# projecthorus/radiosonde_auto_rx

Hardware: AMD Instinct MI355X
Metric: IQ Msamples/s (RS41 --IQ --lpIQ demod + framesync + ECC), concurrent real-time 2.4 Msps channels = value/2.4 (higher is better)
Workload: dtype f32; 1 GPU; RS41 2.4 Msps cs16 IQ, rs41mod --ecc2 --IQ fq --lpIQ (BASELINE configs[1]) x 512 channels per GPU (per-GPU share of configs[4]), 1 s of signal per channel per step, input resident in HBM; channels_per_gpu=512, frames_decoded=507392, frames_ecc_ok=457842, frames_ecc_failed=49550, frames_repaired=200182, symbols_repaired=1815512

## Files before the change

include/sonde_hip.h:

```cpp
#ifndef SONDE_HIP_H
#define SONDE_HIP_H

#include <stdint.h>
#include <stddef.h>

#ifdef __cplusplus
extern "C" {
#endif

#define SONDE_ABI_VERSION 3

#define SONDE_E_ARG      (-1)
#define SONDE_E_NOGPU    (-2)
#define SONDE_E_NOMEM    (-3)
#define SONDE_E_RANGE    (-4)
#define SONDE_E_OVERFLOW (-5)

#define SONDE_RS41  41
#define SONDE_FRONTEND 0
#define SONDE_DFM09  9
#define SONDE_M10    10
#define SONDE_M20    20

#define SONDE_RD94RD41 94
// ... 109 lines not shown
int64_t sonde_engine_samples_to_dc_boundary(const sonde_engine_t *e);
int  sonde_engine_sync(sonde_engine_t *e);

typedef struct {
    uint32_t channel_id;
    uint8_t  type;
    uint8_t  inverted;
    uint16_t reserved;
    float    score;
    float    freq_offset_hz;
    uint64_t sample_pos;
    uint32_t frames;
    uint32_t frames_clean;
} sonde_summary_t;
int  sonde_engine_set_summary(sonde_engine_t *e, void *d_summary, uint32_t channel_base);
int  sonde_engine_set_summary_snapshots(sonde_engine_t *e, void *d_snap);

int  sonde_engine_fetch_frames(sonde_engine_t *e, sonde_frame_t *out, int32_t max);
int  sonde_engine_overflowed(sonde_engine_t *e);
long long sonde_engine_host_ecc_frames(sonde_engine_t *e);
int  sonde_engine_set_device_ecc(sonde_engine_t *e, int32_t on);
int  sonde_engine_set_search_rounds(sonde_engine_t *e, int32_t on);
int  sonde_engine_count_windows(sonde_engine_t *e, int32_t on, int64_t *out);
int  sonde_engine_read_sync_state(sonde_engine_t *e, uint32_t *out, int32_t max_channels);
int  sonde_engine_fetch_frames_lagged(sonde_engine_t *e, sonde_frame_t *out, int32_t max, int32_t lag);

typedef struct {
    int32_t  channel;
    int32_t  nbits;
    uint32_t mv_pos;
    float    mv;
} sonde_hit_t;
int  sonde_engine_fetch_hits(sonde_engine_t *e, sonde_hit_t *out, int32_t max, int32_t finish);
int  sonde_engine_set_sync(sonde_engine_t *e, int32_t hdmax, int32_t bitofs);
int  sonde_engine_fetch_soft1(sonde_engine_t *e, float *soft, int32_t max_frames);
int  sonde_engine_set_threshold(sonde_engine_t *e, float thres);

int  sonde_engine_fetch_dfm(sonde_engine_t *e, sonde_dfm_frame_t *out, int32_t max, int32_t finish);
int  sonde_engine_fetch_dfm_lagged(sonde_engine_t *e, sonde_dfm_frame_t *out, int32_t max, int32_t lag);
typedef struct {
    int32_t  channel;
    int32_t  nbits;
    int32_t  len;
    int32_t  cs_ok;
    uint32_t cs_calc;
    uint32_t mv_pos;
// ... 73 lines not shown
```

radiosonde_auto_rx_amd/csrc/sonde_dev.h:

```cpp
#ifndef SONDE_DEV_H
#define SONDE_DEV_H
#include <hip/hip_runtime.h>
#include <stdint.h>
#include "../../include/sonde_hip.h"

struct MixDecArgs {
    const int16_t *iq;
    long long ch_stride;
    int n_ch, nblocks;
    int D, Q;
    int G;
    int wgs_per_ch;
    float wtab[64 * 8];
    const double *chan_f0;
    int lut_len;
    uint32_t lut_phase;
    const float2 *dc_avg;
    long long *dc_sums;
    const float2 *ptail_in;
    float2 *ptail_out;
    float2 *y;
    int ring_len;
    uint32_t m0;
    const float *wtab_g;
// ... 157 lines not shown
int  sonde_launch_framesync_multi(const SyncArgs *a, int n_groups, hipStream_t s);
int  sonde_launch_mix_decimate(const MixDecArgs *a, hipStream_t s);
void sonde_launch_dc_update(int n_ch, long long *sums, float2 *avg, float maxcnt, hipStream_t s);
void sonde_launch_dc_update_keep(int n_ch, long long *sums, float2 *avg, float2 *avg_prev, float maxcnt, hipStream_t s);
void sonde_launch_publish_u32(const unsigned *src, unsigned *dst_mapped, hipStream_t s);
void sonde_launch_dc_update_pcs(int n_ch, long long *sums, float2 *avg, float2 *avg_prev, uint32_t *cnt, uint32_t *max, uint32_t lim, int32_t *since,
                                uint32_t n_samples, int nblocks, hipStream_t s);
void sonde_launch_md_etable(const double *chan_f0, const float *wtab, int D, int Q, int P, int n_ch, float2 *etab, hipStream_t s);
void sonde_launch_if_chain(const IfArgs *a, hipStream_t s);
void sonde_launch_mix_f32(const MixF32Args *a, hipStream_t s);
void sonde_launch_dc_segments_f32(const float2 *x, long long ch_stride, int n_ch, int n_samples, unsigned dc_cnt0, unsigned dc_max,
                                  double *seg_sums, double *dc_sums, float2 *dc_avg, float2 *dc_seg, int dc_seg_n, hipStream_t s);
void sonde_launch_decimate_f32(const DecF32Args *a, hipStream_t s);
void sonde_launch_dc_update_f64(int n_ch, double *sums, float2 *avg, float maxcnt, hipStream_t s);
void sonde_launch_afc_rotate(const AfcRotArgs *a, hipStream_t s, int n_max);
void sonde_launch_fill_u32(uint32_t *p, uint32_t v, int n, hipStream_t s);
void sonde_launch_audio_chain(const AudioChainArgs *a, hipStream_t s);
void sonde_launch_u8_to_s16(const uint8_t *in, long long in_stride, int16_t *out, long long out_stride, int n_ch, int n_bytes, hipStream_t s);
void sonde_launch_header_corr(const CorrArgs *a, hipStream_t s);
void sonde_launch_sync_plan(const WinPlanArgs *a, hipStream_t s);
void sonde_launch_sync_window_fft(const WinFftArgs *a, hipStream_t s);
void sonde_launch_framesync(const SyncArgs *a, hipStream_t s);
void sonde_launch_search_sync(const SearchSyncArgs *a, hipStream_t s);
}
#endif
```

radiosonde_auto_rx_amd/csrc/sonde_engine.cpp:

```cpp
#include "../../include/sonde_hip.h"
#include "sonde_dev.h"
#include "sonde_host.h"
#include "sonde_scan_dev.h"
#include <algorithm>
#include <cmath>
#include <cstdio>
#include <cstring>
#include <map>
#include <string>
#include <vector>

using namespace sonde;

#define HIPCHK(x) do { hipError_t e_ = (x); if (e_ != hipSuccess) { fprintf(stderr, "libsonde_hip: %s failed: %s\n", #x, hipGetErrorString(e_)); return SONDE_E_NOGPU; } } while (0)

struct KernelStat { double ms = 0; int64_t n = 0; };
struct PendingEvt { hipEvent_t a, b; const char *name; };

struct sonde_engine {
    sonde_cfg_t cfg{};
    sonde_info_t info{};
    hipStream_t stream = nullptr;
    hipStream_t stream_b = nullptr;
    unsigned long long *d_wfprof = nullptr;
// ... 761 lines not shown
            hipMemcpyAsync(e->d_summary_snap + (size_t)(e->call & 1) * C, e->d_summary, (size_t)C * sizeof(sonde_summary_t), hipMemcpyDeviceToDevice, e->stream_b);
            hipEventRecord(e->ev_b[slot], e->stream_b);
            e->snap_calls = e->call + 1;
        }
        e->call += 1;
    } else {
        if (e->stream_b != e->stream) hipEventRecord(e->ev_a[slot], e->stream);
        rc = tail_enqueue(e, n_samples, m_first, e->stream, e->ev_a[slot]);
    }
    return rc;
}

}

static IfArgs fill_if(sonde_engine *e, int n_if, uint32_t m_first) {
    IfArgs b{};
    const bool fe = e->cfg.sonde_type == SONDE_FRONTEND;
    b.y = e->d_y; b.tap_ifiq = (e->cfg.keep_soft || fe) ? e->d_ifiq : nullptr; b.fm = e->d_fm; b.bufs = e->d_bufs; b.n_ch = e->cfg.n_channels; b.ring_len = e->ring_len;
    b.n = n_if; b.m0 = m_first;
    b.lpiq_on = !e->w_iq.empty(); b.lpiq_taps = (int)e->w_iq.size(); b.lpfm_on = !e->w_fm.empty(); b.lpfm_taps = (int)e->w_fm.size();
    b.tone_on = (e->cfg.input != SONDE_IN_IFIQ0); b.nwin = (int)e->sps;
    b.fm_on = (e->cfg.keep_soft || fe || !e->w_fm.empty() || !b.tone_on) ? 1 : 0;
    b.w_iq = e->d_wiq; b.w_fm = e->d_wfm; b.rho = e->rho; b.sps = e->sps; b.epoch = e->d_epoch;
    return b;
}
static int tail_enqueue(sonde_engine *e, int32_t n_samples, uint32_t m_first, hipStream_t fs, hipEvent_t front_done) {
    const int D = e->info.decM, C = e->cfg.n_channels;
    const int n_if = n_samples / D;
    const bool fe = e->cfg.sonde_type == SONDE_FRONTEND;
    IfArgs b = fill_if(e, n_if, m_first);
    const int slot = (int)(e->call & 3);
    if (e->stream_b != fs) hipStreamWaitEvent(e->stream_b, front_done, 0);
    CorrArgs c{};
    c.bufs = e->d_bufs; c.corr = e->d_corr; c.match = e->d_match; c.n_ch = C; c.ring_len = e->ring_len; c.n = n_if; c.L = e->info.L; c.m0 = m_first;
    c.state = e->d_state; c.delay = e->info.delay; c.frame_samples = e->frame_samples;
    c.ntypes = e->corr_types; c.isps = e->corr_isps; c.nsym = e->hdrlen / e->symhd; c.shapes = e->d_shapes; c.sym_type = e->d_symtype; c.sym_sign = e->d_symsign;
    if (e->cfg.opt_dc && e->cfg.input != SONDE_IN_AUDIO) {
        hipStream_t sb = e->stream_b;
        sonde_launch_fill_u32(e->d_start, m_first, C, sb);
        b.y = e->d_yrot; b.tap_ifiq = e->d_ifiq; b.afc = e->d_afc; b.start = e->d_start; b.fmraw = e->d_fmraw; b.w_iq0 = e->d_wiq0; b.fm_on = 1;
        c.start = e->d_start;
        AfcRotArgs r{}; r.y = e->d_y; r.yrot = e->d_yrot; r.afc = e->d_afc; r.start = e->d_start; r.n_ch = C; r.ring_len = e->ring_len;
        r.sr = e->info.if_sr; r.m_end = e->m_out;
        for (int it = 0; it < n_if / std::max(1, e->info.K - 4) + 4; it++) {
            hipMemsetAsync(e->d_pending, 0, sizeof(unsigned), sb);
            sonde_launch_afc_rotate(&r, sb, n_if);
            prof_begin(e, "if_chain", sb); sonde_launch_if_chain(&b, sb); prof_end(e, sb);
            prof_begin(e, "header_corr", sb); sonde_launch_header_corr(&c, sb); prof_end(e, sb);
            if (e->opt_iq >= 2) { CorrArgs c2 = c; c2.bufs = e->d_fm; c2.corr = e->d_corr2; sonde_launch_header_corr(&c2, sb); }
            launch_framesync(e, 0);
            hipMemcpyAsync(e->h_pending, e->d_pending, sizeof(unsigned), hipMemcpyDeviceToHost, sb);
            HIPCHK(hipStreamSynchronize(sb));
            if (*e->h_pending == 0) break;
        }
        if (e->stream_b != fs) hipEventRecord(e->ev_if[slot], e->stream_b);
    } else {
        if (e->cfg.input != SONDE_IN_AUDIO) { prof_begin(e, "if_chain", e->stream_b); sonde_launch_if_chain(&b, e->stream_b); prof_end(e, e->stream_b); }
        if (e->stream_b != fs) hipEventRecord(e->ev_if[slot], e->stream_b);
        if (!fe && e->d_win && !e->search_rounds) {
            launch_search_sync(e);
        } else if (!fe && e->d_win) {
            const int rounds = sync_rounds_of(e, n_if);
            for (int round = 0; round < rounds; round++) {
// ... 217 lines not shown
    if (!e) return SONDE_E_ARG;
    long long n = e->host_ecc_frames;
    for (sonde_engine *g : e->groups) n += g->host_ecc_frames;
    return n;
}
int sonde_engine_set_search_rounds(sonde_engine_t *e, int32_t on) {
    if (!e) return SONDE_E_ARG;
    for (sonde_engine *g : e->groups) { const int rc = sonde_engine_set_search_rounds(g, on); if (rc) return rc; }
    e->search_rounds = on != 0;
    return 0;
}
int sonde_engine_count_windows(sonde_engine_t *e, int32_t on, int64_t *out) {
    if (!e || !e->groups.empty()) return SONDE_E_ARG;
    if (on && !e->d_wcount && e->d_win && dalloc(&e->d_wcount, 1)) return SONDE_E_NOMEM;
    if (hipStreamSynchronize(e->stream_b) != hipSuccess) return SONDE_E_NOGPU;
    e->count_windows = on != 0;
    if (out) {
        unsigned long long n = 0;
        if (e->d_wcount && hipMemcpy(&n, e->d_wcount, sizeof n, hipMemcpyDeviceToHost) != hipSuccess) return SONDE_E_NOGPU;
        out[0] = e->wcount_rounds[0]; out[1] = e->wcount_rounds[1]; out[2] = (int64_t)n;
    }
    return 0;
}
int sonde_engine_read_sync_state(sonde_engine_t *e, uint32_t *out, int32_t max_channels) {
    if (!e || !out || !e->groups.empty() || !e->d_state) return SONDE_E_ARG;
    const int n = std::min<int>(max_channels, e->cfg.n_channels);
    if (n <= 0) return 0;
    if (hipStreamSynchronize(e->stream_b) != hipSuccess) return SONDE_E_NOGPU;
    if (hipMemcpy(out, e->d_state, (size_t)n * sizeof(SyncState), hipMemcpyDeviceToHost) != hipSuccess) return SONDE_E_NOGPU;
    return n;
}
int sonde_engine_set_device_ecc(sonde_engine_t *e, int32_t on) {
    if (!e) return SONDE_E_ARG;
    for (sonde_engine *g : e->groups) { const int rc = sonde_engine_set_device_ecc(g, on); if (rc) return rc; }
    if ((on != 0) == e->dev_ecc) return 0;
    if (e->d_blk_done) {
        if (hipStreamSynchronize(e->stream_b) != hipSuccess) return SONDE_E_NOGPU;
        unsigned count = 0;
        if (hipMemcpy(&count, e->d_fcount, sizeof count, hipMemcpyDeviceToHost) != hipSuccess) return SONDE_E_NOGPU;
        if (count != e->read_idx) return SONDE_E_ARG;
        const unsigned dn[2] = { count, 0u };
        if (on && hipMemcpy(e->d_blk_done, dn, sizeof dn, hipMemcpyHostToDevice) != hipSuccess) return SONDE_E_NOGPU;
    }
    e->dev_ecc = on != 0;
    return 0;
}
// ... 478 lines not shown
```

radiosonde_auto_rx_amd/csrc/sonde_kernels.hip:

```cpp
#include <hip/hip_runtime.h>
#include <stdint.h>
#include "sonde_dev.h"
#include "md_fast_gen.h"
#include "sonde_rs_dev.h"
#include <cstdlib>

typedef short  short2v __attribute__((ext_vector_type(2)));

#define WAVE 64

#define MD_ROWS   64
#define MD_NVMAX  16

struct __attribute__((packed, aligned(4))) u32x4_u { uint32_t x, y, z, w; };

typedef float float2v __attribute__((ext_vector_type(2)));

__device__ __forceinline__ float2v cmul_pk(float2v u, float2v cs) {
    float2v t, z;
    asm("s_nop 0\n\tv_pk_mul_f32 %0, %1, %2 op_sel:[1,1] op_sel_hi:[1,0] neg_lo:[0,1]" : "=&v"(t) : "v"(u), "v"(cs));
    asm("v_pk_fma_f32 %0, %1, %2, %3 op_sel_hi:[0,1,1]" : "=&v"(z) : "v"(u), "v"(cs), "v"(t));
    return z;
}

template <int Q_T, bool WRAP, bool PH64>
__device__ __forceinline__ void md_step(const uint32_t raw, const int r, const float *w, const float2v navg, const float2v msk,
                                        const double f0, double &ndrun, const uint32_t rown, const uint32_t towrap, const uint32_t L,
                                        float2v (&acc)[Q_T], float2v &dcs) {
// ... 1031 lines not shown
        yr[m & mask] = r;
    }
}

__global__ void k_fill_u32(uint32_t *p, uint32_t v, int n) {
    const int i = blockIdx.x * blockDim.x + threadIdx.x;
    if (i < n) p[i] = v;
}

#ifndef IF_TILE
#define IF_TILE 960
#endif
#ifndef IF_THREADS
#define IF_THREADS 256
#endif
#ifndef IF_NB
#define IF_NB 4
#endif
#define IF_RUN 4
#ifndef IF_LD
#define IF_LD 5
#endif

__device__ __forceinline__ void if_chain_body(const IfArgs &a, const int ch, const int bx) {
    extern __shared__ __attribute__((aligned(16))) float smem[];
    const uint32_t t0 = a.m0 + (uint32_t)bx * IF_TILE;
    const int nout = min(IF_TILE, (int)(a.m0 + (uint32_t)a.n - t0));
    if (nout <= 0) return;
    const bool afc = a.afc != nullptr;
    const uint32_t start = afc ? a.start[ch] : t0;
    if (afc && (int32_t)(t0 + (uint32_t)nout - start) <= 0) return;
    const uint32_t mask = (uint32_t)a.ring_len - 1;
    const int T1 = a.lpiq_on ? a.lpiq_taps : 1;
    const int T2 = a.lpfm_on ? a.lpfm_taps : 1;
    const int nwin = a.nwin;
    const int64_t ep = a.epoch ? (int64_t)a.epoch[ch] : 0;
    const int hz = (T2 - 1) + max(1, nwin - 1);
    const int nz = hz + nout;
    const int ny = nz + (T1 - 1);
    const int nyp = (ny + 2 * IF_NB + 1) & ~1;
    float2 *sy = reinterpret_cast<float2 *>(smem);
    const int nzs = a.fm_on ? nz + (nz & 1) : 0;
    float2 *sz = sy + nyp;
    float4 *sx4 = reinterpret_cast<float4 *>(sz + nzs);
    float  *sf = reinterpret_cast<float *>(sx4 + (a.tone_on ? nz : 0));
    const int nsf = a.fm_on ? T2 - 1 + nout : 0;
    float  *wf = sf + nsf;
    float  *wq = sf + ((nsf + T2 + 3) & ~3);

    const float2 *yr = a.y + (size_t)ch * a.ring_len;
    for (int kb = threadIdx.x; kb < nyp; kb += IF_LD * IF_THREADS) {
        float2 v[IF_LD];
#pragma unroll
        for (int u = 0; u < IF_LD; u++) {
            const int k = kb + u * IF_THREADS;
            const int64_t m = (int64_t)t0 - hz - (T1 - 1) + k;
            v[u] = (m >= 0 && k < ny) ? yr[(uint32_t)m & mask] : make_float2(0.f, 0.f);
        }
#pragma unroll
        for (int u = 0; u < IF_LD; u++) { const int k = kb + u * IF_THREADS; if (k < nyp) sy[k] = v[u]; }
    }
    const int acq = __builtin_amdgcn_readfirstlane((afc && !a.afc[ch].locked) ? 1 : 0);
    const float *w_iq = acq ? a.w_iq0 : a.w_iq;
    for (int k = threadIdx.x; k < T2; k += IF_THREADS) wf[k] = a.lpfm_on ? a.w_fm[k] : 1.0f;
    for (int k = threadIdx.x; k < T1; k += IF_THREADS) wq[k] = a.lpiq_on ? w_iq[k] : 1.0f;
    typedef const float __attribute__((address_space(4))) *cfptr;
    const cfptr wtaps = (cfptr)(uintptr_t)w_iq;
    __syncthreads();

    typedef float v2f __attribute__((ext_vector_type(2)));
    for (int k0 = IF_NB * threadIdx.x; k0 < nz; k0 += IF_NB * IF_THREADS) {
        v2f acc[IF_NB];
#pragma unroll
        for (int j = 0; j < IF_NB; j++) acc[j] = v2f{0.f, 0.f};
        v2f win[IF_NB + 2];
#pragma unroll
        for (int j = 0; j < IF_NB; j += 2) {
            const float4 v0 = *reinterpret_cast<const float4 *>(sy + k0 + j);
            win[j] = v2f{v0.x, v0.y}; win[j + 1] = v2f{v0.z, v0.w};
        }
        int t = 0;
#ifdef IF_EXP_NOFIR
        t = T1 & ~3;
#endif
        for (; t + 3 < T1; t += 4) {
            const float4 n0 = *reinterpret_cast<const float4 *>(sy + k0 + t + IF_NB), n1 = *reinterpret_cast<const float4 *>(sy + k0 + t + IF_NB + 2);
            const float4 w4 = make_float4(wtaps[t], wtaps[t + 1], wtaps[t + 2], wtaps[t + 3]);
            win[IF_NB] = v2f{n0.x, n0.y}; win[IF_NB + 1] = v2f{n0.z, n0.w};
#pragma unroll
            for (int j = 0; j < IF_NB; j++) {
                acc[j] = __builtin_elementwise_fma(win[j], v2f{w4.x, w4.x}, acc[j]);
                acc[j] = __builtin_elementwise_fma(win[j + 1], v2f{w4.y, w4.y}, acc[j]);
            }
// ... 29 lines not shown
#pragma unroll
            for (int j = 0; j < IF_NB; j++) acc[j] = __builtin_elementwise_fma(win[j], v2f{w0, w0}, acc[j]);
        }
#pragma unroll
        for (int j = 0; j < IF_NB; j++) {
            const int k = k0 + j;
            if (k >= nz) break;
            float re = acc[j].x, im = acc[j].y;
            const int64_t m = (int64_t)t0 - hz + k;
            if (m < 0) { re = 0.f; im = 0.f; }
            else if (afc && (int32_t)((uint32_t)m - start) < 0) {
                const float2 zo = a.tap_ifiq[(size_t)ch * a.ring_len + ((uint32_t)m & mask)];
                re = zo.x; im = zo.y;
            }
            if (a.fm_on) sz[k] = make_float2(re, im);
            if (a.tone_on) {
#ifdef IF_EXP_NOTONE
                const float sn = 0.f, cs = 1.f;
#else
                const float fr = (float)__builtin_amdgcn_fract((double)(m - ep) * a.rho);
                const float sn = __builtin_amdgcn_sinf(fr), cs = __builtin_amdgcn_cosf(fr);
#endif
                const float rc = re * cs, ic = im * cs;
                sx4[k] = make_float4(__builtin_fmaf(-sn, im, rc), __builtin_fmaf(sn, re, ic), __builtin_fmaf(sn, im, rc), __builtin_fmaf(-sn, re, ic));
            }
            if (a.tap_ifiq && m >= (int64_t)t0 && (int32_t)((uint32_t)m - start) >= 0)
                a.tap_ifiq[(size_t)ch * a.ring_len + ((uint32_t)m & mask)] = make_float2(re, im);
        }
    }
    __syncthreads();

    if (a.fm_on)
    for (int k = threadIdx.x; k < T2 - 1 + nout; k += IF_THREADS) {
        const int zi = k + (hz - (T2 - 1));
        const float2 z1 = sz[zi], z0 = sz[zi - 1];
        const float wr = z1.x * z0.x + z1.y * z0.y, wi = z1.y * z0.x - z1.x * z0.y;
#ifdef IF_EXP_NOATAN
        float v = wi + wr;
#else
        float v = 0.8f * atan2f(wi, wr) * 0.31830988618379067f;
#endif
        if (afc) {
            const int64_t m = (int64_t)t0 - (T2 - 1) + k;
            float *fr = a.fmraw + (size_t)ch * a.ring_len;
            if (m >= 0 && (int32_t)((uint32_t)m - start) < 0) v = fr[(uint32_t)m & mask];
            else if (m >= (int64_t)t0) fr[(uint32_t)m & mask] = v;
        }
        sf[k] = v;
    }
    __syncthreads();

    float *bufs = a.bufs + (size_t)ch * a.ring_len;
    float *fmb = a.fm + (size_t)ch * a.ring_len;
    const float inv_sps = 1.0f / a.sps;
    for (int k0 = IF_RUN * threadIdx.x; k0 < nout; k0 += IF_RUN * IF_THREADS) {
        float4 f = make_float4(0.f, 0.f, 0.f, 0.f);
        float so[IF_RUN], sfm[IF_RUN];
        const bool vec = !afc && k0 + IF_RUN <= nout && ((t0 + (uint32_t)k0) & (IF_RUN - 1)) == 0;
#pragma unroll
        for (int r = 0; r < IF_RUN; r++) {
            const int k = k0 + r;
            so[r] = 0.f; sfm[r] = 0.f;
            if (k >= nout) break;
            const uint32_t m = t0 + (uint32_t)k;
            if (a.tone_on) {
#ifdef IF_EXP_NOWIN
                if (1) { f = sx4[hz + k]; } else
#endif
                if (r == 0) {
                    for (int j = nwin - 1; j >= 0; j--) { const float4 x = sx4[hz + k - j]; f.x += x.x; f.y += x.y; f.z += x.z; f.w += x.w; }
                } else {
                    const float4 xn = sx4[hz + k], xo = sx4[hz + k - nwin];
                    f.x += xn.x - xo.x; f.y += xn.y - xo.y; f.z += xn.z - xo.z; f.w += xn.w - xo.w;
                }
            }
            if (afc && (int32_t)(m - start) < 0) continue;
            float s_fm = 0.f;
            if (a.fm_on) {
                s_fm = sf[T2 - 1 + k];
                if (a.lpfm_on) {
                    float acc = 0.f;
                    for (int t = 0; t < T2; t++) acc = fmaf(sf[k + t], wf[t], acc);
                    s_fm = acc;
                }
                if (!vec) fmb[m & mask] = s_fm;
            }
            float s = s_fm;
            if (a.tone_on) s = (__builtin_amdgcn_sqrtf(f.z * f.z + f.w * f.w) - __builtin_amdgcn_sqrtf(f.x * f.x + f.y * f.y)) * inv_sps;
            if (!vec) bufs[m & mask] = s;
            so[r] = s; sfm[r] = s_fm;
        }
        if (vec) {
            const uint32_t mi = (t0 + (uint32_t)k0) & mask;
            static_assert(IF_RUN == 4, "the vector store below writes four outputs");
            *reinterpret_cast<float4 *>(bufs + mi) = make_float4(so[0], so[1], so[2], so[3]);
            if (a.fm_on) *reinterpret_cast<float4 *>(fmb + mi) = make_float4(sfm[0], sfm[1], sfm[2], sfm[3]);
        }
    }
}

__global__ __launch_bounds__(IF_THREADS)
void k_if_chain(const IfArgs a) { if_chain_body(a, blockIdx.y, blockIdx.x); }
template <class A> struct MultiArgs { A g[SONDE_MAX_GROUPS]; int row0[SONDE_MAX_GROUPS + 1]; int n_groups; };
template <class A> __device__ __forceinline__ int multi_group(const MultiArgs<A> &m, const int row) {
    int g = 0;
    while (g + 1 < m.n_groups && row >= m.row0[g + 1]) g++;
    return __builtin_amdgcn_readfirstlane(g);
}
__global__ __launch_bounds__(IF_THREADS)
void k_if_chain_multi(const MultiArgs<IfArgs> m) {
    const int g = multi_group(m, (int)blockIdx.y);
    if_chain_body(m.g[g], (int)blockIdx.y - m.row0[g], blockIdx.x);
}

__device__ __forceinline__ uint32_t sync_first_pos(const SyncState &st, uint32_t frame_samples, int delay) {
    uint32_t first;
    if (st.mode == 1) first = st.mv_pos + 1 + frame_samples;
    else first = st.s_in - st.k;
    return first - (uint32_t)(delay + 16);
}
__device__ __forceinline__ bool corr_tile_unused(const CorrArgs &a, int ch, uint32_t tile_start, uint32_t tile_end) {
    if (a.start && (int32_t)(tile_end - a.start[ch]) <= 0) return true;
    if (!a.state) return false;
    const SyncState st = a.state[ch];
    if (st.mode != 0 && st.mode != 1) return true;
    const uint32_t first = sync_first_pos(st, a.frame_samples, a.delay);
    if (a.limit && (int32_t)(tile_start - (first + a.limit)) >= 0) return true;
    return (int32_t)(tile_end - first) <= 0;
}

#define HC_TILE 1024
#define HC_THREADS 256
// ... 83 lines not shown
    float *corr = a.corr + (size_t)ch * a.ring_len;
#if HCF_TILE / HCF_THREADS >= 2
    for (int o2 = threadIdx.x * 2; o2 < HCF_TILE; o2 += 2 * HCF_THREADS) {
        float c0 = 0.f, c1 = 0.f;
        for (int k = 0; k < nsym; k++) {
            const int ty = a.sym_type[k];
            const float sg = a.sym_sign[k];
            const float2 u = *reinterpret_cast<const float2 *>(sF + ty * nf + sps * k + o2);
            c0 = fmaf(sg, u.x, c0); c1 = fmaf(sg, u.y, c1);
        }
        if (o2 < nout) corr[(p0 + (uint32_t)o2) & mask] = c0;
        if (o2 + 1 < nout) corr[(p0 + (uint32_t)(o2 + 1)) & mask] = c1;
    }
#else
    {
        const int o = threadIdx.x;
        float c0 = 0.f;
        for (int k = 0; k < nsym; k++) c0 = fmaf(a.sym_sign[k], sF[a.sym_type[k] * nf + sps * k + o], c0);
        if (o < nout) corr[(p0 + (uint32_t)o) & mask] = c0;
    }
#endif
}

__device__ __forceinline__ float wave_sum(float v) {
    for (int off = 32; off > 0; off >>= 1) v += __shfl_xor(v, off);
    return v;
}

__device__ __forceinline__ void bit_window(int pos, int half, int symlen, float sps,
                                           uint32_t &q0, uint32_t &q1, double &mid) {
    double bg = (pos == 0) ? 0.0 : (double)((float)(pos * symlen) * sps);
    double prev;
    if (half == 0) {
        if (pos == 0) prev = 0.0;
        else {
            prev = (pos == 1) ? 0.0 : (double)((float)((pos - 1) * symlen) * sps);
            prev += (double)sps;
            if (symlen == 2) prev += (double)sps;
        }
    } else {
        bg += (double)sps;
        prev = bg;
    }
    q0 = (uint32_t)ceil(prev);
    mid = bg + (double)(sps - 1.0f) / 2.0;
    q1 = (uint32_t)ceil(bg + (double)sps);
// ... 90 lines not shown
    __syncthreads();
    float c = corr[mpos & mask];
    if (DC) c -= off;
    mv = c / sqrtf(e);
    return bidx;
}

struct NoWinEval {
    static constexpr bool fused = false;
    __device__ int operator()(int, uint32_t, float &, uint32_t &) const { return -4; }
};
template <bool DC, int NT = FS_THREADS, class Eval = NoWinEval>
__device__ __forceinline__ void framesync_body(const SyncArgs &a, const int ch, const Eval &eval = Eval{}) {
    __shared__ uint8_t s_frame[520];
    __shared__ uint8_t s_exp[512];
    __shared__ uint8_t s_log[256];
    __shared__ float s_rf[(NT / WAVE)];
    __shared__ int s_ri[(NT / WAVE)];
    __shared__ int s_cnt[2];
    __shared__ unsigned s_slot;
    __shared__ uint8_t s_syn[(NT / WAVE)][48];
    __shared__ uint8_t s_S[48];
    __shared__ double s_rd[(NT / WAVE)];
    const int tid = threadIdx.x, lane = tid & 63, wave = tid >> 6;
    if (ch >= a.n_ch) return;
    const uint32_t mask = (uint32_t)a.ring_len - 1;
    const float *bufs = a.bufs + (size_t)ch * a.ring_len;
    const float *corr = a.corr + (size_t)ch * a.ring_len;
    SyncState st = a.state[ch];
    const uint32_t ep = a.epoch ? a.epoch[ch] : 0u;
    uint32_t avail = a.avail;
    AfcState af{};
    if (DC) af = a.afc[ch];
    bool afc_event = false;
    const int K = a.K, L = a.L;

#define FS_MARK(k) do { if (a.prof && ch == 0 && tid == 0) { const unsigned long long t_ = __builtin_readcyclecounter(); a.prof[k] += t_ - t_prev; t_prev = t_; } } while (0)
    unsigned long long t_prev = a.prof ? __builtin_readcyclecounter() : 0ull;
    for (int i = tid; i < 512; i += NT) s_exp[i] = a.gf_exp[i];
    for (int i = tid; i < 256; i += NT) s_log[i] = a.gf_log[i];
    __syncthreads();
    FS_MARK(0);
    const bool horizon_on = a.corr_limit != 0 && (st.mode == 0 || st.mode == 1);
    const uint32_t horizon = horizon_on ? sync_first_pos(st, a.frame_samples, a.delay) + a.corr_limit : 0u;

    for (int guard = 0; guard < (1 << 20); guard++) {
        if (st.mode == 2) break;
        if (st.mode == 0) {
            const uint32_t need = (uint32_t)(K - 4) - st.k;
            const uint32_t s_in_w = st.s_in + need;
            if ((int32_t)(avail - s_in_w) < 0) { st.k += avail - st.s_in; st.s_in = avail; break; }
            if (horizon_on && (int32_t)(s_in_w - 1 - (uint32_t)a.delay - horizon) >= 0) break;
            const uint32_t pos = s_in_w - 1 - (uint32_t)a.delay;
            const WinItem *wi = nullptr;
            if (!DC && !Eval::fused && a.win && pos >= (uint32_t)L) {
                for (int w = 0; w < a.win_W; w++) { const WinItem *c = a.win + (size_t)ch * a.win_W + w; if (c->state == 2 && c->pos == pos) { wi = c; break; } }
                if (!wi) break;
            }
            st.s_in = s_in_w; st.k = 0; st.mv = 0.f;
            if (pos - ep < (uint32_t)L) continue;
            float mv; uint32_t mpos;
            if (wi) { if (wi->rc < 0) { if (wi->rc == -5) st.mv_pos = wi->mpos; continue; } mv = wi->mv; mpos = wi->mpos; }
            else if (Eval::fused && pos >= (uint32_t)L) {
                const int rc = eval(ch, pos, mv, mpos);
                if (rc < 0) { if (rc == -5) st.mv_pos = mpos; continue; }
            } else {
                const int rc = fs_window<DC, NT>(bufs, corr, mask, pos, K, L, a.N, a.match_sum, tid, lane, wave, s_rf, s_ri, mv, mpos);
                if (rc == -5) { st.mv_pos = mpos; if (DC) af.dc = 0.0; }
                if (rc < 0) continue;
            }
// ... 263 lines not shown
#define WF_THREADS 512
#endif
#define FFT_THREADS WF_THREADS
#include "sonde_fft_dev.h"
#ifndef WF_MB
#define WF_MB 4
#endif
#ifndef WF_LU
#define WF_LU 1
#endif
#ifndef WF_LB
#define WF_LB 4
#endif
#define WF_MARK(k) do { if (a.prof && blockIdx.x == 0 && tid == 0) { const unsigned long long t_ = __builtin_readcyclecounter(); a.prof[k] += t_ - t_prev; t_prev = t_; } } while (0)
struct WinItemIo {
    static constexpr int copy = 0;
    WinItem *it;
    __device__ bool planned() const { return it->state == 1; }
    __device__ uint32_t pos() const { return it->pos; }
    __device__ void put(int rc, float mv, uint32_t mpos) const { it->rc = rc; it->mv = mv; it->mpos = mpos; __threadfence(); it->state = 2; }
};
template <class Io>
__device__ __forceinline__ void sync_eval_window(const WinFftArgs &a, const int ch, const Io &io, float2 *x, float2 *tws, float *s_rf, int *s_ri) {
    const int tid = threadIdx.x, lane = tid & 63, wave = tid >> 6;
    if (!io.planned()) return;
    unsigned long long t_prev = a.prof ? __builtin_readcyclecounter() : 0ull;
    const int K = a.K, L = a.L, N = SC_N, wl = K + L;
    const uint32_t pos = io.pos(), mask = (uint32_t)a.ring_len - 1;
    const float *bufs = a.bufs + (size_t)ch * a.ring_len;
    const int64_t start = (int64_t)pos - (wl - 1);
    {
        constexpr int NL = SC_N / WF_THREADS;
#pragma unroll 1
        for (int h = 0; h < NL; h += WF_LB) {
            float v[WF_LB];
#pragma unroll
            for (int u = 0; u < WF_LB; u++) {
                const int i = tid + (h + u) * WF_THREADS;
                const int64_t p = start + i;
                v[u] = (i < wl && p >= 0) ? bufs[(uint32_t)p & mask] : 0.f;
            }
#pragma unroll
            for (int u = 0; u < WF_LB; u++) x[XI(brev13(tid + (h + u) * WF_THREADS))] = make_float2(v[u], 0.f);
        }
    }
    __syncthreads();
    WF_MARK(0);
    dft_ref<Io::copy>(x, tws, a.tws, tid);
    WF_MARK(1);
    {
        const float2 *FmR = a.Fm + N;
#pragma unroll 1
        for (int h = 0; h < N / WF_THREADS; h += WF_MB) {
            float2 fi[WF_MB], fr[WF_MB];
#pragma unroll
            for (int u = 0; u < WF_MB; u++) {
                const int i = tid + (h + u) * WF_THREADS;
                const bool on = brev13(i) >= i;
                fi[u] = on ? a.Fm[i] : make_float2(0.f, 0.f);
                fr[u] = on ? FmR[i] : make_float2(0.f, 0.f);
            }
#pragma unroll
            for (int u = 0; u < WF_MB; u++) {
                const int i = tid + (h + u) * WF_THREADS, r = brev13(i);
                if (r < i) continue;
                const float2 zi = cmul(x[XI(i)], fi[u]), zr = cmul(x[XI(r)], fr[u]);
                x[XI(r)] = make_float2(zi.x, -zi.y);
                x[XI(i)] = make_float2(zr.x, -zr.y);
            }
        }
    }
    __syncthreads();
    WF_MARK(2);
    dft_ref_head<Io::copy>(x, tws, a.tws, tid);
    float best = 0.f, bestc = 0.f; int bidx = -1;
#pragma unroll WF_LU
    for (int u = 0; u < SC_N / 2 / WF_THREADS; u++) {
        const int g = tid + u * WF_THREADS;
        const float2 w = a.tws[((1 << 12) - 1) + g];
        const float2 p = x[XI(g)], r = cmul(x[XI(g + (1 << 12))], w);
        const float c0 = p.x + r.x, c1 = p.x - r.x;
        const int i0 = g, i1 = g + (1 << 12);
        if (i0 >= L - 1 && i0 < wl) { const float c2 = c0 * c0; if (c2 > best || (c2 == best && bidx >= 0 && i0 < bidx)) { best = c2; bidx = i0; bestc = c0; } }
        if (i1 >= L - 1 && i1 < wl) { const float c2 = c1 * c1; if (c2 > best || (c2 == best && bidx >= 0 && i1 < bidx)) { best = c2; bidx = i1; bestc = c1; } }
    }
    WF_MARK(3);
    {
        float rb = best; int ri = bidx;
        for (int off = 32; off > 0; off >>= 1) {
            const float ob = __shfl_xor(rb, off); const int oi = __shfl_xor(ri, off);
            if (ob > rb || (ob == rb && oi >= 0 && (ri < 0 || oi < ri))) { rb = ob; ri = oi; }
        }
        if (lane == 0) { s_rf[wave] = rb; s_ri[wave] = ri; }
    }
    __syncthreads();
    int mp = -1;
// ... 215 lines not shown
extern "C" void sonde_launch_decimate_f32(const DecF32Args *a, hipStream_t s) {
    if (a->nblocks <= 0) return;
    int jper = DF32_J;
    auto lds_of = [&](int j) { return (size_t)(a->D * (j - 1) + a->T) * sizeof(float2) + (size_t)a->T * sizeof(float); };
    while (jper > 8 && lds_of(jper) > 64 * 1024) jper >>= 1;
    if (lds_of(jper) > 64 * 1024) { hipLaunchKernelGGL(k_decimate_f32_global, dim3((a->nblocks + 255) / 256, a->n_ch), dim3(256), 0, s, *a); return; }
    hipLaunchKernelGGL(k_decimate_f32, dim3((a->nblocks + jper - 1) / jper, a->n_ch), dim3(DF32_J), lds_of(jper), s, *a, jper);
}
extern "C" void sonde_launch_dc_update_f64(int n_ch, double *sums, float2 *avg, float maxcnt, hipStream_t s) {
    hipLaunchKernelGGL(k_dc_update_f64, dim3((n_ch + 255) / 256), dim3(256), 0, s, n_ch, sums, avg, maxcnt);
}
extern "C" void sonde_launch_afc_rotate(const AfcRotArgs *a, hipStream_t s, int n_max) {
    int gx = (n_max + 255) / 256; if (gx > 256) gx = 256; if (gx < 1) gx = 1;
    hipLaunchKernelGGL(k_afc_rotate, dim3(gx, a->n_ch), dim3(256), 0, s, *a);
}
extern "C" void sonde_launch_fill_u32(uint32_t *p, uint32_t v, int n, hipStream_t s) {
    hipLaunchKernelGGL(k_fill_u32, dim3((n + 255) / 256), dim3(256), 0, s, p, v, n);
}
extern "C" void sonde_launch_audio_chain(const AudioChainArgs *a, hipStream_t s) {
    int gx = (a->n + 255) / 256; if (gx > 256) gx = 256; if (gx < 1) gx = 1;
    hipLaunchKernelGGL(k_audio_chain, dim3(gx, a->n_ch), dim3(256), 0, s, *a);
}
extern "C" void sonde_launch_if_chain(const IfArgs *a, hipStream_t s) {
    const int T1 = a->lpiq_on ? a->lpiq_taps : 1, T2 = a->lpfm_on ? a->lpfm_taps : 1;
    const int hz = (T2 - 1) + (a->nwin - 1 > 1 ? a->nwin - 1 : 1);
    const int nz = hz + IF_TILE, ny = nz + T1 - 1;
    const size_t lds = (size_t)((ny + 2 * IF_NB + 1) & ~1) * 8 + (size_t)(a->fm_on ? nz + 1 : 0) * 8 + (size_t)(a->tone_on ? nz : 0) * 16 + (size_t)(a->fm_on ? T2 - 1 + IF_TILE : 0) * 4 + (size_t)(T1 + T2) * 4 + 32;
    hipLaunchKernelGGL(k_if_chain, dim3((a->n + IF_TILE - 1) / IF_TILE, a->n_ch), dim3(IF_THREADS), lds, s, *a);
}
template <class A> static MultiArgs<A> multi_pack(const A *a, const int *rows, int n_groups) {
    MultiArgs<A> m{};
    m.n_groups = n_groups; m.row0[0] = 0;
    for (int g = 0; g < n_groups; g++) { m.g[g] = a[g]; m.row0[g + 1] = m.row0[g] + rows[g]; }
    return m;
}
static_assert(sizeof(MultiArgs<IfArgs>) <= 4096, "MultiArgs<IfArgs> exceeds the kernel argument segment");
static_assert(sizeof(MultiArgs<WinPlanArgs>) <= 4096, "MultiArgs<WinPlanArgs> exceeds the kernel argument segment");
static_assert(sizeof(MultiArgs<WinFftArgs>) <= 4096, "MultiArgs<WinFftArgs> exceeds the kernel argument segment");
static_assert(sizeof(MultiArgs<SyncArgs>) <= 4096, "MultiArgs<SyncArgs> exceeds the kernel argument segment");
extern "C" int sonde_launch_if_chain_multi(const IfArgs *a, int n_groups, hipStream_t s) {
    if (n_groups < 1 || n_groups > SONDE_MAX_GROUPS) return -1;
    size_t lds = 0; int rows[SONDE_MAX_GROUPS], n = a[0].n;
    for (int g = 0; g < n_groups; g++) {
        const int T1 = a[g].lpiq_on ? a[g].lpiq_taps : 1, T2 = a[g].lpfm_on ? a[g].lpfm_taps : 1;
        const int hz = (T2 - 1) + (a[g].nwin - 1 > 1 ? a[g].nwin - 1 : 1);
        const int nz = hz + IF_TILE, ny = nz + T1 - 1;
        const size_t l = (size_t)((ny + 2 * IF_NB + 1) & ~1) * 8 + (size_t)(a[g].fm_on ? nz + 1 : 0) * 8 + (size_t)(a[g].tone_on ? nz : 0) * 16 + (size_t)(a[g].fm_on ? T2 - 1 + IF_TILE : 0) * 4 + (size_t)(T1 + T2) * 4 + 32;
        if (l > lds) lds = l;
        rows[g] = a[g].n_ch;
        if (a[g].n != n) return -1;
    }
    const MultiArgs<IfArgs> m = multi_pack(a, rows, n_groups);
    hipLaunchKernelGGL(k_if_chain_multi, dim3((n + IF_TILE - 1) / IF_TILE, m.row0[n_groups]), dim3(IF_THREADS), lds, s, m);
    return 0;
}
extern "C" int sonde_launch_sync_plan_multi(const WinPlanArgs *a, int n_groups, hipStream_t s) {
    if (n_groups < 1 || n_groups > SONDE_MAX_GROUPS) return -1;
    int rows[SONDE_MAX_GROUPS];
    for (int g = 0; g < n_groups; g++) rows[g] = a[g].n_ch;
    const MultiArgs<WinPlanArgs> m = multi_pack(a, rows, n_groups);
    hipLaunchKernelGGL(k_sync_plan_multi, dim3((m.row0[n_groups] + 255) / 256), dim3(256), 0, s, m);
    return 0;
}
extern "C" int sonde_launch_sync_window_fft_multi(const WinFftArgs *a, int n_groups, hipStream_t s) {
    if (n_groups < 1 || n_groups > SONDE_MAX_GROUPS) return -1;
    long long tot = 0; int rows[SONDE_MAX_GROUPS];
    for (int g = 0; g < n_groups; g++) tot += (long long)a[g].W * a[g].n_ch;
    const long long cap = tot > 512 ? 512 : tot;
    for (int g = 0; g < n_groups; g++) { const long long w = (long long)a[g].W * a[g].n_ch; rows[g] = (int)((w * cap + tot - 1) / tot); if (rows[g] < 1) rows[g] = 1; }
    const MultiArgs<WinFftArgs> m = multi_pack(a, rows, n_groups);
// ... 78 lines not shown
    if (tid == 0) { ecc[f] = r; codes[2 * f] = L.res[0]; codes[2 * f + 1] = L.res[1]; }
}
extern "C" void sonde_launch_rs41_ecc_batch(uint8_t *frames, const int32_t *flen, int n, int level, int32_t *ecc, int32_t *codes, uint8_t *synd,
                                            const uint8_t *gf_exp, const uint8_t *gf_log, hipStream_t s) {
    hipLaunchKernelGGL(k_rs41_ecc_batch, dim3(n), dim3(RSK_THREADS), 0, s, frames, flen, level, ecc, codes, synd, gf_exp, gf_log, (const unsigned *)nullptr);
}
extern "C" void sonde_launch_rs41_ecc_batch_n(uint8_t *frames, const int32_t *flen, const unsigned *count, int cap, int level, int32_t *ecc, int32_t *codes, uint8_t *synd,
                                              const uint8_t *gf_exp, const uint8_t *gf_log, hipStream_t s) {
    hipLaunchKernelGGL(k_rs41_ecc_batch, dim3(cap), dim3(RSK_THREADS), 0, s, frames, flen, level, ecc, codes, synd, gf_exp, gf_log, count);
}

extern "C" int sonde_launch_framesync_multi(const SyncArgs *a, int n_groups, hipStream_t s) {
    if (n_groups < 1 || n_groups > SONDE_MAX_GROUPS) return -1;
    int rows[SONDE_MAX_GROUPS];
    for (int g = 0; g < n_groups; g++) { rows[g] = a[g].n_ch; if (a[g].opt_dc) return -1; }
    const MultiArgs<SyncArgs> m = multi_pack(a, rows, n_groups);
    hipLaunchKernelGGL(k_framesync_multi, dim3(m.row0[n_groups]), dim3(1024), 0, s, m);
    return 0;
}
extern "C" void sonde_launch_framesync(const SyncArgs *a, hipStream_t s) {
    if (a->opt_dc) hipLaunchKernelGGL(k_framesync<true>, dim3(a->n_ch), dim3(FS_THREADS), 0, s, *a);
    else hipLaunchKernelGGL(k_framesync<false>, dim3(a->n_ch), dim3(FS_THREADS), 0, s, *a);
}
extern "C" void sonde_launch_search_sync(const SearchSyncArgs *a, hipStream_t s) {
    const size_t lds = (size_t)(SC_XN + SC_TW_LDS + 1) * sizeof(float2);
    hipLaunchKernelGGL(k_search_sync, dim3(a->sync.n_ch), dim3(WF_THREADS), lds, s, *a);
}
```

radiosonde_auto_rx_amd/engine.py:

```python
from __future__ import annotations

import ctypes as C
import os
import subprocess

import numpy as np

_HERE = os.path.dirname(os.path.abspath(__file__))
LIB_PATH = os.environ.get("SONDE_HIP_LIB", os.path.join(_HERE, "libsonde_hip.so"))

SONDE_RS41 = 41
SONDE_DFM09 = 9
SONDE_M10 = 10
SONDE_RD94RD41 = 94
SONDE_M20 = 20
LP_IQ, LP_FM = 1, 2
TAP_DECIM, TAP_IFIQ, TAP_FM, TAP_BUFS, TAP_CORR = range(5)
ABI_VERSION = 3


class SondeCfg(C.Structure):
    _fields_ = [(n, C.c_int32) for n in ("abi_version", "device", "n_channels", "sample_rate", "bits", "sonde_type",
                                         "opt_lp", "opt_dc", "opt_min", "lpiq_bw", "ecc_level")] + \
               [("thres", C.c_float), ("max_chunk", C.c_int32), ("max_frames", C.c_int32), ("keep_soft", C.c_int32),
# ... 199 lines not shown
    def set_summary(self, device_ptr: int, channel_base: int = 0):
        _chk(lib().sonde_engine_set_summary(self._h, C.c_void_p(device_ptr), channel_base))

    def set_summary_snapshots(self, device_ptr: int) -> int:
        return _chk(lib().sonde_engine_set_summary_snapshots(self._h, C.c_void_p(device_ptr)))

    def overflowed(self) -> bool:
        return bool(_chk(lib().sonde_engine_overflowed(self._h)))

    def host_ecc_frames(self) -> int:
        return int(lib().sonde_engine_host_ecc_frames(self._h))

    def set_device_ecc(self, on: bool):
        _chk(lib().sonde_engine_set_device_ecc(self._h, 1 if on else 0))

    def set_search_rounds(self, on: bool):
        _chk(lib().sonde_engine_set_search_rounds(self._h, 1 if on else 0))

    def count_windows(self, on: bool = True):
        out = np.zeros(3, dtype=np.int64)
        _chk(lib().sonde_engine_count_windows(self._h, 1 if on else 0, out.ctypes.data))
        return {"round0": int(out[0]), "rounds": int(out[1]), "search_sync": int(out[2])}

    def sync_state(self) -> np.ndarray:
        out = np.zeros((self.n_channels, 8), dtype=np.uint32)
        _chk(lib().sonde_engine_read_sync_state(self._h, out.ctypes.data, self.n_channels))
        return out

    def fetch_frames(self, max_frames: int | None = None, with_soft: bool = False, finish: bool = False):
        n = max_frames or self._max_frames
        buf = (SondeFrame * n)()
        fn = lib().sonde_engine_finish if finish else lib().sonde_engine_fetch_frames
        k = _chk(fn(self._h, buf, n))
        frames = []
        line = C.create_string_buffer(1200)
        for i in range(k):
            f = buf[i]
            ll = lib().sonde_rs41_rawline(C.byref(f), line, 1200)
            frames.append(dict(channel=f.channel, len=f.len, ecc=f.ecc, mv=f.mv, mv_pos=f.mv_pos, nbytes=f.nbytes,
                               frame=bytes(f.frame), line=line.raw[:ll].decode()))
        if with_soft:
            soft = np.zeros((max(k, 1), self.nbits), np.float32)
            _chk(lib().sonde_engine_fetch_soft(self._h, soft.ctypes.data_as(C.c_void_p), k))
            for i in range(k):
                frames[i]["soft"] = soft[i].copy()
        return frames
# ... 141 lines not shown
```

Measured before the change: 913,700 Msamples/s.

## Overlay IF-chain LDS buffers and pin waves-per-EU to raise occupancy

The IF-chain kernel can now overlay the tone float4 buffer onto the input/sz region when the tone window fits. Tone samples are held in registers until the FM stage is done and are then stored. This shrinks the kernel's LDS footprint, and the kernel also gets amdgpu_waves_per_eu(8,8) plus an SGPR cap, all aimed at more resident blocks per CU. WF_FRESH asm barriers are added in search_sync and framesync to stop derived thread indices being kept live in registers, and a residency query API is exposed. The risks are register spills under the forced wave limit and an extra barrier.

```diff
diff --git a/include/sonde_hip.h b/include/sonde_hip.h
--- a/include/sonde_hip.h
+++ b/include/sonde_hip.h
@@ -155,6 +155,7 @@
 int  sonde_engine_set_device_ecc(sonde_engine_t *e, int32_t on);
 int  sonde_engine_set_search_rounds(sonde_engine_t *e, int32_t on);
 int  sonde_engine_count_windows(sonde_engine_t *e, int32_t on, int64_t *out);
+int  sonde_engine_tail_residency(sonde_engine_t *e, int32_t *out);
 int  sonde_engine_read_sync_state(sonde_engine_t *e, uint32_t *out, int32_t max_channels);
 int  sonde_engine_fetch_frames_lagged(sonde_engine_t *e, sonde_frame_t *out, int32_t max, int32_t lag);
 
diff --git a/radiosonde_auto_rx_amd/csrc/sonde_dev.h b/radiosonde_auto_rx_amd/csrc/sonde_dev.h
--- a/radiosonde_auto_rx_amd/csrc/sonde_dev.h
+++ b/radiosonde_auto_rx_amd/csrc/sonde_dev.h
@@ -203,5 +203,7 @@
 void sonde_launch_sync_window_fft(const WinFftArgs *a, hipStream_t s);
 void sonde_launch_framesync(const SyncArgs *a, hipStream_t s);
 void sonde_launch_search_sync(const SearchSyncArgs *a, hipStream_t s);
+int  sonde_if_chain_residency(const IfArgs *a);
+int  sonde_search_sync_residency(void);
 }
 #endif
diff --git a/radiosonde_auto_rx_amd/csrc/sonde_engine.cpp b/radiosonde_auto_rx_amd/csrc/sonde_engine.cpp
--- a/radiosonde_auto_rx_amd/csrc/sonde_engine.cpp
+++ b/radiosonde_auto_rx_amd/csrc/sonde_engine.cpp
@@ -807,6 +807,7 @@
     b.tone_on = (e->cfg.input != SONDE_IN_IFIQ0); b.nwin = (int)e->sps;
     b.fm_on = (e->cfg.keep_soft || fe || !e->w_fm.empty() || !b.tone_on) ? 1 : 0;
     b.w_iq = e->d_wiq; b.w_fm = e->d_wfm; b.rho = e->rho; b.sps = e->sps; b.epoch = e->d_epoch;
+    if (e->cfg.opt_dc && e->cfg.input != SONDE_IN_AUDIO) b.fm_on = 1;
     return b;
 }
 static int tail_enqueue(sonde_engine *e, int32_t n_samples, uint32_t m_first, hipStream_t fs, hipEvent_t front_done) {
@@ -823,7 +824,7 @@
     if (e->cfg.opt_dc && e->cfg.input != SONDE_IN_AUDIO) {
         hipStream_t sb = e->stream_b;
         sonde_launch_fill_u32(e->d_start, m_first, C, sb);
-        b.y = e->d_yrot; b.tap_ifiq = e->d_ifiq; b.afc = e->d_afc; b.start = e->d_start; b.fmraw = e->d_fmraw; b.w_iq0 = e->d_wiq0; b.fm_on = 1;
+        b.y = e->d_yrot; b.tap_ifiq = e->d_ifiq; b.afc = e->d_afc; b.start = e->d_start; b.fmraw = e->d_fmraw; b.w_iq0 = e->d_wiq0;
         c.start = e->d_start;
         AfcRotArgs r{}; r.y = e->d_y; r.yrot = e->d_yrot; r.afc = e->d_afc; r.start = e->d_start; r.n_ch = C; r.ring_len = e->ring_len;
         r.sr = e->info.if_sr; r.m_end = e->m_out;
@@ -1087,6 +1088,13 @@
     }
     return 0;
 }
+int sonde_engine_tail_residency(sonde_engine_t *e, int32_t *out) {
+    if (!e || !out || !e->groups.empty()) return SONDE_E_ARG;
+    const IfArgs b = fill_if(e, 0, 0);
+    out[0] = e->cfg.input != SONDE_IN_AUDIO ? sonde_if_chain_residency(&b) : 0;
+    out[1] = (e->cfg.sonde_type != SONDE_FRONTEND && e->d_win && !e->cfg.opt_dc) ? sonde_search_sync_residency() : 0;
+    return (out[0] < 0 || out[1] < 0) ? SONDE_E_NOGPU : 0;
+}
 int sonde_engine_read_sync_state(sonde_engine_t *e, uint32_t *out, int32_t max_channels) {
     if (!e || !out || !e->groups.empty() || !e->d_state) return SONDE_E_ARG;
     const int n = std::min<int>(max_channels, e->cfg.n_channels);
diff --git a/radiosonde_auto_rx_amd/csrc/sonde_kernels.hip b/radiosonde_auto_rx_amd/csrc/sonde_kernels.hip
--- a/radiosonde_auto_rx_amd/csrc/sonde_kernels.hip
+++ b/radiosonde_auto_rx_amd/csrc/sonde_kernels.hip
@@ -4,6 +4,7 @@
 #include "md_fast_gen.h"
 #include "sonde_rs_dev.h"
 #include <cstdlib>
+#include <algorithm>
 
 typedef short  short2v __attribute__((ext_vector_type(2)));
 
@@ -1081,6 +1082,16 @@
 #define IF_LD 5
 #endif
 
+__host__ __device__ __forceinline__ int  if_chain_xlo(int T2) { return (T2 - 1) & ~(IF_NB - 1); }
+__host__ __device__ __forceinline__ bool if_chain_overlay(int tone_on, int T2, int hz) { return tone_on && hz + IF_TILE - if_chain_xlo(T2) <= IF_NB * IF_THREADS; }
+static size_t if_chain_lds(const IfArgs &a) {
+    const int T1 = a.lpiq_on ? a.lpiq_taps : 1, T2 = a.lpfm_on ? a.lpfm_taps : 1, hz = (T2 - 1) + std::max(1, a.nwin - 1);
+    const int nz = hz + IF_TILE, ny = nz + T1 - 1, nsf = a.fm_on ? T2 - 1 + IF_TILE : 0;
+    const size_t sy = (size_t)((ny + 2 * IF_NB + 1) & ~1) * 8, sz = (size_t)(a.fm_on ? nz + 1 : 0) * 8, tail = (size_t)(T1 + T2) * 4 + 32;
+    if (if_chain_overlay(a.tone_on, T2, hz)) return std::max(sy + sz, (size_t)((nsf + 3) & ~3) * 4 + (size_t)(nz - if_chain_xlo(T2)) * 16) + tail;
+    return sy + sz + (size_t)(a.tone_on ? nz : 0) * 16 + (size_t)nsf * 4 + tail;
+}
+
 __device__ __forceinline__ void if_chain_body(const IfArgs &a, const int ch, const int bx) {
     extern __shared__ __attribute__((aligned(16))) float smem[];
     const uint32_t t0 = a.m0 + (uint32_t)bx * IF_TILE;
@@ -1101,11 +1112,13 @@
     float2 *sy = reinterpret_cast<float2 *>(smem);
     const int nzs = a.fm_on ? nz + (nz & 1) : 0;
     float2 *sz = sy + nyp;
-    float4 *sx4 = reinterpret_cast<float4 *>(sz + nzs);
-    float  *sf = reinterpret_cast<float *>(sx4 + (a.tone_on ? nz : 0));
+    const bool ovl = if_chain_overlay(a.tone_on, T2, hz);
+    const int xlo = ovl ? if_chain_xlo(T2) : 0;
     const int nsf = a.fm_on ? T2 - 1 + nout : 0;
-    float  *wf = sf + nsf;
-    float  *wq = sf + ((nsf + T2 + 3) & ~3);
+    float  *sf = ovl ? smem : reinterpret_cast<float *>(sz + nzs) + (a.tone_on ? 4 * nz : 0);
+    float4 *sx4 = ovl ? reinterpret_cast<float4 *>(smem + ((nsf + 3) & ~3)) : reinterpret_cast<float4 *>(sz + nzs);
+    float  *wf = ovl ? smem + max(2 * nyp + 2 * nzs, ((nsf + 3) & ~3) + 4 * (nz - xlo)) : sf + nsf;
+    float  *wq = ovl ? wf + ((T2 + 3) & ~3) : sf + ((nsf + T2 + 3) & ~3);
 
     const float2 *yr = a.y + (size_t)ch * a.ring_len;
     for (int kb = threadIdx.x; kb < nyp; kb += IF_LD * IF_THREADS) {
@@ -1128,6 +1141,7 @@
     __syncthreads();
 
     typedef float v2f __attribute__((ext_vector_type(2)));
+    float4 xr[IF_NB]; int xk0 = -1;
     for (int k0 = IF_NB * threadIdx.x; k0 < nz; k0 += IF_NB * IF_THREADS) {
         v2f acc[IF_NB];
 #pragma unroll
@@ -1203,7 +1217,9 @@
                 const float sn = __builtin_amdgcn_sinf(fr), cs = __builtin_amdgcn_cosf(fr);
 #endif
                 const float rc = re * cs, ic = im * cs;
-                sx4[k] = make_float4(__builtin_fmaf(-sn, im, rc), __builtin_fmaf(sn, re, ic), __builtin_fmaf(sn, im, rc), __builtin_fmaf(-sn, re, ic));
+                const float4 x4 = make_float4(__builtin_fmaf(-sn, im, rc), __builtin_fmaf(sn, re, ic), __builtin_fmaf(sn, im, rc), __builtin_fmaf(-sn, re, ic));
+                if (!ovl) sx4[k] = x4;
+                else if (k0 >= xlo) { xr[j] = x4; xk0 = k0; }
             }
             if (a.tap_ifiq && m >= (int64_t)t0 && (int32_t)((uint32_t)m - start) >= 0)
                 a.tap_ifiq[(size_t)ch * a.ring_len + ((uint32_t)m & mask)] = make_float2(re, im);
@@ -1229,6 +1245,13 @@
         }
         sf[k] = v;
     }
+    if (ovl) {
+        if (a.fm_on) __syncthreads();
+        if (xk0 >= 0) {
+#pragma unroll
+            for (int j = 0; j < IF_NB; j++) { const int k = xk0 + j; if (k < nz) sx4[k - xlo] = xr[j]; }
+        }
+    }
     __syncthreads();
 
     float *bufs = a.bufs + (size_t)ch * a.ring_len;
@@ -1246,12 +1269,12 @@
             const uint32_t m = t0 + (uint32_t)k;
             if (a.tone_on) {
 #ifdef IF_EXP_NOWIN
-                if (1) { f = sx4[hz + k]; } else
+                if (1) { f = sx4[hz + k - xlo]; } else
 #endif
                 if (r == 0) {
-                    for (int j = nwin - 1; j >= 0; j--) { const float4 x = sx4[hz + k - j]; f.x += x.x; f.y += x.y; f.z += x.z; f.w += x.w; }
+                    for (int j = nwin - 1; j >= 0; j--) { const float4 x = sx4[hz + k - xlo - j]; f.x += x.x; f.y += x.y; f.z += x.z; f.w += x.w; }
                 } else {
-                    const float4 xn = sx4[hz + k], xo = sx4[hz + k - nwin];
+                    const float4 xn = sx4[hz + k - xlo], xo = sx4[hz + k - xlo - nwin];
                     f.x += xn.x - xo.x; f.y += xn.y - xo.y; f.z += xn.z - xo.z; f.w += xn.w - xo.w;
                 }
             }
@@ -1280,7 +1303,10 @@
     }
 }
 
-__global__ __launch_bounds__(IF_THREADS)
+#ifndef IF_WAVES_ATTR
+#define IF_WAVES_ATTR __attribute__((amdgpu_waves_per_eu(8, 8), amdgpu_num_sgpr(96)))
+#endif
+__global__ __launch_bounds__(IF_THREADS) IF_WAVES_ATTR
 void k_if_chain(const IfArgs a) { if_chain_body(a, blockIdx.y, blockIdx.x); }
 template <class A> struct MultiArgs { A g[SONDE_MAX_GROUPS]; int row0[SONDE_MAX_GROUPS + 1]; int n_groups; };
 template <class A> __device__ __forceinline__ int multi_group(const MultiArgs<A> &m, const int row) {
@@ -1288,7 +1314,7 @@
     while (g + 1 < m.n_groups && row >= m.row0[g + 1]) g++;
     return __builtin_amdgcn_readfirstlane(g);
 }
-__global__ __launch_bounds__(IF_THREADS)
+__global__ __launch_bounds__(IF_THREADS) IF_WAVES_ATTR
 void k_if_chain_multi(const MultiArgs<IfArgs> m) {
     const int g = multi_group(m, (int)blockIdx.y);
     if_chain_body(m.g[g], (int)blockIdx.y - m.row0[g], blockIdx.x);
@@ -1418,6 +1444,7 @@
 #endif
 }
 
+#define WF_FRESH(t) asm volatile("" : "+v"(t))
 __device__ __forceinline__ float wave_sum(float v) {
     for (int off = 32; off > 0; off >>= 1) v += __shfl_xor(v, off);
     return v;
@@ -1554,7 +1581,7 @@
     __shared__ uint8_t s_syn[(NT / WAVE)][48];
     __shared__ uint8_t s_S[48];
     __shared__ double s_rd[(NT / WAVE)];
-    const int tid = threadIdx.x, lane = tid & 63, wave = tid >> 6;
+    int tid = threadIdx.x;
     if (ch >= a.n_ch) return;
     const uint32_t mask = (uint32_t)a.ring_len - 1;
     const float *bufs = a.bufs + (size_t)ch * a.ring_len;
@@ -1578,6 +1605,8 @@
 
     for (int guard = 0; guard < (1 << 20); guard++) {
         if (st.mode == 2) break;
+        WF_FRESH(tid);
+        const int lane = tid & 63, wave = tid >> 6;
         if (st.mode == 0) {
             const uint32_t need = (uint32_t)(K - 4) - st.k;
             const uint32_t s_in_w = st.s_in + need;
@@ -1887,7 +1916,9 @@
 };
 template <class Io>
 __device__ __forceinline__ void sync_eval_window(const WinFftArgs &a, const int ch, const Io &io, float2 *x, float2 *tws, float *s_rf, int *s_ri) {
-    const int tid = threadIdx.x, lane = tid & 63, wave = tid >> 6;
+    int tid = threadIdx.x;
+    WF_FRESH(tid);
+    const int lane = tid & 63, wave = tid >> 6;
     if (!io.planned()) return;
     unsigned long long t_prev = a.prof ? __builtin_readcyclecounter() : 0ull;
     const int K = a.K, L = a.L, N = SC_N, wl = K + L;
@@ -1911,8 +1942,10 @@
     }
     __syncthreads();
     WF_MARK(0);
+    WF_FRESH(tid);
     dft_ref<Io::copy>(x, tws, a.tws, tid);
     WF_MARK(1);
+    WF_FRESH(tid);
     {
         const float2 *FmR = a.Fm + N;
 #pragma unroll 1
@@ -1937,6 +1970,7 @@
     }
     __syncthreads();
     WF_MARK(2);
+    WF_FRESH(tid);
     dft_ref_head<Io::copy>(x, tws, a.tws, tid);
     float best = 0.f, bestc = 0.f; int bidx = -1;
 #pragma unroll WF_LU
@@ -2198,11 +2232,7 @@
     hipLaunchKernelGGL(k_audio_chain, dim3(gx, a->n_ch), dim3(256), 0, s, *a);
 }
 extern "C" void sonde_launch_if_chain(const IfArgs *a, hipStream_t s) {
-    const int T1 = a->lpiq_on ? a->lpiq_taps : 1, T2 = a->lpfm_on ? a->lpfm_taps : 1;
-    const int hz = (T2 - 1) + (a->nwin - 1 > 1 ? a->nwin - 1 : 1);
-    const int nz = hz + IF_TILE, ny = nz + T1 - 1;
-    const size_t lds = (size_t)((ny + 2 * IF_NB + 1) & ~1) * 8 + (size_t)(a->fm_on ? nz + 1 : 0) * 8 + (size_t)(a->tone_on ? nz : 0) * 16 + (size_t)(a->fm_on ? T2 - 1 + IF_TILE : 0) * 4 + (size_t)(T1 + T2) * 4 + 32;
-    hipLaunchKernelGGL(k_if_chain, dim3((a->n + IF_TILE - 1) / IF_TILE, a->n_ch), dim3(IF_THREADS), lds, s, *a);
+    hipLaunchKernelGGL(k_if_chain, dim3((a->n + IF_TILE - 1) / IF_TILE, a->n_ch), dim3(IF_THREADS), if_chain_lds(*a), s, *a);
 }
 template <class A> static MultiArgs<A> multi_pack(const A *a, const int *rows, int n_groups) {
     MultiArgs<A> m{};
@@ -2218,10 +2248,7 @@
     if (n_groups < 1 || n_groups > SONDE_MAX_GROUPS) return -1;
     size_t lds = 0; int rows[SONDE_MAX_GROUPS], n = a[0].n;
     for (int g = 0; g < n_groups; g++) {
-        const int T1 = a[g].lpiq_on ? a[g].lpiq_taps : 1, T2 = a[g].lpfm_on ? a[g].lpfm_taps : 1;
-        const int hz = (T2 - 1) + (a[g].nwin - 1 > 1 ? a[g].nwin - 1 : 1);
-        const int nz = hz + IF_TILE, ny = nz + T1 - 1;
-        const size_t l = (size_t)((ny + 2 * IF_NB + 1) & ~1) * 8 + (size_t)(a[g].fm_on ? nz + 1 : 0) * 8 + (size_t)(a[g].tone_on ? nz : 0) * 16 + (size_t)(a[g].fm_on ? T2 - 1 + IF_TILE : 0) * 4 + (size_t)(T1 + T2) * 4 + 32;
+        const size_t l = if_chain_lds(a[g]);
         if (l > lds) lds = l;
         rows[g] = a[g].n_ch;
         if (a[g].n != n) return -1;
@@ -2346,7 +2373,15 @@
     if (a->opt_dc) hipLaunchKernelGGL(k_framesync<true>, dim3(a->n_ch), dim3(FS_THREADS), 0, s, *a);
     else hipLaunchKernelGGL(k_framesync<false>, dim3(a->n_ch), dim3(FS_THREADS), 0, s, *a);
 }
+static constexpr size_t SEARCH_SYNC_LDS = (size_t)(SC_XN + SC_TW_LDS + 1) * sizeof(float2);
 extern "C" void sonde_launch_search_sync(const SearchSyncArgs *a, hipStream_t s) {
-    const size_t lds = (size_t)(SC_XN + SC_TW_LDS + 1) * sizeof(float2);
-    hipLaunchKernelGGL(k_search_sync, dim3(a->sync.n_ch), dim3(WF_THREADS), lds, s, *a);
-}
+    hipLaunchKernelGGL(k_search_sync, dim3(a->sync.n_ch), dim3(WF_THREADS), SEARCH_SYNC_LDS, s, *a);
+}
+extern "C" int sonde_if_chain_residency(const IfArgs *a) {
+    int n = 0;
+    return hipOccupancyMaxActiveBlocksPerMultiprocessor(&n, k_if_chain, IF_THREADS, if_chain_lds(*a)) == hipSuccess ? n : -1;
+}
+extern "C" int sonde_search_sync_residency(void) {
+    int n = 0;
+    return hipOccupancyMaxActiveBlocksPerMultiprocessor(&n, k_search_sync, WF_THREADS, SEARCH_SYNC_LDS) == hipSuccess ? n : -1;
+}
diff --git a/radiosonde_auto_rx_amd/engine.py b/radiosonde_auto_rx_amd/engine.py
--- a/radiosonde_auto_rx_amd/engine.py
+++ b/radiosonde_auto_rx_amd/engine.py
@@ -245,6 +245,13 @@
         _chk(lib().sonde_engine_count_windows(self._h, 1 if on else 0, out.ctypes.data))
         return {"round0": int(out[0]), "rounds": int(out[1]), "search_sync": int(out[2])}
 
+    def tail_residency(self):
+        out = np.zeros(2, dtype=np.int32)
+        f = lib().sonde_engine_tail_residency
+        f.argtypes = [C.c_void_p, C.c_void_p]
+        _chk(f(self._h, out.ctypes.data))
+        return {"if_chain": int(out[0]), "search_sync": int(out[1])}
+
     def sync_state(self) -> np.ndarray:
         out = np.zeros((self.n_channels, 8), dtype=np.uint32)
         _chk(lib().sonde_engine_read_sync_state(self._h, out.ctypes.data, self.n_channels))
```

Result: faster. 934,500 Msamples/s, median of 6 (+2.3%).
